# ndpp/ndpp

Hardware: AMD Instinct MI355X
Metric: E_in points*Legendre-orders/sec (free-gas scatter moments) (higher is better)
Workload: dtype f64

## Files before the change

ndpp_amd/csrc/fg_device.h:

```cpp
#pragma once

#include <hip/hip_runtime.h>

#include "fg_pipeline.h"

namespace ndpp {
namespace {

constexpr int kWave = 64;
constexpr int kMuWavesPerSimd = 2;
constexpr int kMuBlocksPerCU = 4 * kMuWavesPerSimd;

struct DevAtomics {
  __device__ static int add(int* p, int v) { return atomicAdd(p, v); }
};

typedef __attribute__((address_space(3))) double lds_f64;
typedef __attribute__((address_space(3))) unsigned lds_u32;

constexpr int mu_stack_fields(int R) { return 2 + 2 * R; }
constexpr int mu_lds_levels(int R) {
  const int budget = (160 * 1024) / kMuBlocksPerCU - 64;
  const int fit = budget / (kWave * (8 * mu_stack_fields(R) + 4));
  return (R == 1 && fit > kStackLdsLevels) ? kStackLdsLevels : fit;
}

template <int R>
struct DevMuStack {
  static constexpr int NF = mu_stack_fields(R);
  lds_f64* lds;
  lds_u32* ldsm;
  char* gbase;
  unsigned goff, gstride;
  int lane, d0;
  static constexpr unsigned kRecBytes = 8u * (NF + 1);
  __device__ __forceinline__ bool in_lds(int d) const { return d >= d0; }
  __device__ __forceinline__ void push(int d, double b, double w, const double* Xb,
                                       const double* Xe, unsigned m) {
    if (in_lds(d)) {
      const int o = __mul24(d - d0, NF * kWave) + lane;
      lds[o] = b; lds[o + kWave] = w;
#pragma unroll
      for (int r = 0; r < R; ++r) {
        lds[o + (2 + r) * kWave] = Xb[r];
        lds[o + (2 + R + r) * kWave] = Xe[r];
      }
      ldsm[(d - d0) * kWave + lane] = m;
    } else {
      double* p = (double*)(gbase + (size_t)(goff + __umul24((unsigned)d, gstride)));
      p[0] = b; p[1] = w;
#pragma unroll
      for (int r = 0; r < R; ++r) { p[2 + r] = Xb[r]; p[2 + R + r] = Xe[r]; }
      *(unsigned*)(p + NF) = m;
    }
  }
  __device__ __forceinline__ void pop(int d, double& b, double& w, double* Xb,
                                      double* Xe, unsigned& m) const {
    if (in_lds(d)) {
      const int o = __mul24(d - d0, NF * kWave) + lane;
      b = lds[o]; w = lds[o + kWave];
#pragma unroll
      for (int r = 0; r < R; ++r) {
        Xb[r] = lds[o + (2 + r) * kWave];
        Xe[r] = lds[o + (2 + R + r) * kWave];
      }
      m = ldsm[(d - d0) * kWave + lane];
    } else {
      const double* p = (const double*)(gbase + (size_t)(goff + __umul24((unsigned)d, gstride)));
      b = p[0]; w = p[1];
#pragma unroll
      for (int r = 0; r < R; ++r) { Xb[r] = p[2 + r]; Xe[r] = p[2 + R + r]; }
      m = *(const unsigned*)(p + NF);
    }
  }
};

__global__ void fg_prep_kernel(FgBatch B, int level) {
  if (*B.overflow) return;
  const int base = B.lvl_off(level);
  const int nt = B.n_tasks(level);
  for (int t = blockIdx.x * blockDim.x + threadIdx.x; t < nt;
       t += gridDim.x * blockDim.x)
    fg_prep_task(B, level, base, t);
}

template <int R, int LMAX, bool kPath>
__device__ __forceinline__ void mu_wave_loop(const FgBatch& B, int level, int base, int nt,
                                             int* counter, DevMuStack<R>& st) {
  MuLane<R, LMAX> s;
  s.mask = 0;
  const PnConsts pk = make_pn_consts<(R * LMAX <= 12 && LMAX <= 8)>();
  bool active = false, more = true;
  bool counts = true;
  unsigned long long n_k = 0, n_v = 0, n_i = 0, n_o = 0;
  unsigned long long w_it = 0, l_it = 0;
  const int kTaskBlock = nt >= (int)(gridDim.x * 16 * kWave) ? 4 * kWave : kWave;
  int blk_next = 0, blk_end = 0;
  constexpr int kFetchMin = kPath ? 8 : 1;
  auto lanes = [](bool x) -> unsigned long long { return __builtin_amdgcn_ballot_w64(x); };
  for (;;) {
    unsigned long long need = more ? lanes(!active) : 0ull;
    if (kFetchMin > 1 && need && __popcll(need) < kFetchMin && lanes(active)) need = 0;
    if (need) {
      if (blk_next >= blk_end) {
        const int first = __ffsll((long long)need) - 1;
        int b = 0;
        if (threadIdx.x == (unsigned)first) b = atomicAdd(counter, kTaskBlock);
        b = __builtin_amdgcn_readlane(b, first);
        blk_next = b;
        blk_end = (b + kTaskBlock < nt) ? b + kTaskBlock : nt;
        if (b >= nt) more = false;
      }
      if (!active && more) {
        const int rank = __popcll(need & ((1ull << threadIdx.x) - 1ull));
        const int t = blk_next + rank;
        if (t < blk_end) {
          if (kPath) mu_init_split<R, LMAX>(B, level, base, t, s);
          else mu_init<R, LMAX>(B, level, base, t, s);
          active = (s.mask != 0);
          if (kPath) counts = (s.path_bits == 0);
          if (active) mu_tot_zero(s);
        }
      }
      const int taken = __popcll(need);
      blk_next = (blk_next + taken < blk_end) ? blk_next + taken : blk_end;
    }
    const unsigned long long act = lanes(active);
    if (!act && !more) break;
    w_it += 1;
    l_it += (unsigned long long)__popcll(act);
    if (active) {
      if (!mu_step<R, LMAX, DevMuStack<R>, kPath>(B, s, st, pk)) {
        mu_finish(B, s, kPath);
        n_k += 2ull * s.visits + 3;
        n_v += s.visits;
        n_o += s.ovisits;
        n_i += counts ? 1 : 0;
        active = false;
      }
    }
  }
  for (int o = 32; o > 0; o >>= 1) {
    n_k += __shfl_down(n_k, o);
    n_v += __shfl_down(n_v, o);
    n_i += __shfl_down(n_i, o);
    n_o += __shfl_down(n_o, o);
  }
  if (threadIdx.x == 0) {
    atomicAdd(&B.stats[kStatKEvals], n_k);
    atomicAdd(&B.stats[kStatMuVisits], n_v);
    atomicAdd(&B.stats[kStatMuIntegrals], n_i);
    atomicAdd(&B.stats[kStatOrderVisits], n_o);
    atomicAdd(&B.stats[kStatWaveIters], w_it);
    atomicAdd(&B.stats[kStatLaneIters], l_it);
  }
}

template <int R, int LMAX>
__global__ __launch_bounds__(kWave, kMuWavesPerSimd) void fg_mu_kernel(FgBatch B, int level, double* gstack, int* counter) {
  constexpr int NF = mu_stack_fields(R), kLevels = mu_lds_levels(R);
  __shared__ double lds[kLevels * NF * kWave];
  __shared__ unsigned ldsm[kLevels * kWave];
  DevMuStack<R> st;
  st.lds = (lds_f64*)lds;
  st.ldsm = (lds_u32*)ldsm;
  st.gbase = (char*)gstack;
  st.goff = (blockIdx.x * kWave + threadIdx.x) * DevMuStack<R>::kRecBytes;
  st.gstride = gridDim.x * kWave * DevMuStack<R>::kRecBytes;
  st.lane = threadIdx.x;
  st.d0 = B.mu_its > kLevels ? B.mu_its - kLevels : 0;

  if (*B.overflow) return;
  const int base = B.lvl_off(level);
  if (B.split_level(level))
    mu_wave_loop<R, LMAX, true>(B, level, base, B.n_mu_tasks(level) * kSplit, counter, st);
  else
    mu_wave_loop<R, LMAX, false>(B, level, base, B.n_mu_tasks(level), counter, st);
}

__global__ void fg_seg_zero_kernel(FgBatch B, int level) {
  if (*B.overflow || !B.split_level(level)) return;
  const size_t n = (size_t)B.n_mu_tasks(level) * kSplit * B.nch();
  for (size_t k = blockIdx.x * (size_t)blockDim.x + threadIdx.x; k < n; k += (size_t)gridDim.x * blockDim.x)
    B.seg[k] = 0.0;
}

__global__ void fg_mu_combine_kernel(FgBatch B, int level) {
  if (*B.overflow || !B.split_level(level)) return;
  const int base = B.lvl_off(level);
  const int nch = B.nch();
  const long tot = (long)B.n_mu_tasks(level) * nch;
  for (long k = blockIdx.x * (long)blockDim.x + threadIdx.x; k < tot; k += (long)gridDim.x * blockDim.x) {
    const int t = (int)(k / nch), ch = (int)(k - (long)t * nch);
    int n, slot;
    fg_task_decode(B, level, base, t, n, slot);
    const unsigned mask = (unsigned)B.node_info[4 * n + 0];
    const int r = ch / B.L, l = ch - r * B.L;
    if (!(mask & chan_bit(r, l))) continue;
    const unsigned gl_rows = B.t_gl ? B.t_gl[B.rec_index(level, base, n, slot)] : 0u;
    if (gl_rows >> r & 1u) continue;
    const double* sg = B.seg + (size_t)t * kSplit * nch + ch;
    double sum = 0.0;
    for (int j = 0; j < kSplit; ++j) sum = sum + sg[(size_t)j * nch];
    B.F(slot, ch, n) = sum;
  }
}

__global__ void fg_setup_kernel(FgBatch B) {
  const int n = B.n_jobs * B.G;
  for (int i = blockIdx.x * blockDim.x + threadIdx.x; i < n;
       i += gridDim.x * blockDim.x)
    fg_setup_group(B, i / B.G, i % B.G);
}

__global__ void fg_node_kernel(FgBatch B, int level) {
  if (*B.overflow) return;
  const int base = B.lvl_off(level);
  const int nn = B.lvl_cnt[level];
  for (int i = blockIdx.x * blockDim.x + threadIdx.x; i < nn;
       i += gridDim.x * blockDim.x)
    fg_node_process<DevAtomics>(B, level, base, i);
  if (blockIdx.x == 0 && threadIdx.x == 0)
    atomicAdd(&B.stats[kStatEoutNodes], (unsigned long long)nn);
}

__global__ void fg_reduce_kernel(FgBatch B, int level) {
  if (*B.overflow) return;
  const int base = B.lvl_off(level);
  const int nn = B.lvl_cnt[level];
  for (int i = blockIdx.x * blockDim.x + threadIdx.x; i < nn;
       i += gridDim.x * blockDim.x)
    fg_reduce_node(B, base, i);
}

__global__ void fg_assemble_kernel(FgBatch B) {
  if (*B.overflow) return;
  const int n_calls = B.n_jobs * B.R;
  for (int c = blockIdx.x * blockDim.x + threadIdx.x; c < n_calls;
       c += gridDim.x * blockDim.x)
    fg_assemble_call(B, c);
}

inline int fg_blocks(long n, int threads = 256) {
  long b = (n + threads - 1) / threads;
  return (int)(b < 1 ? 1 : (b > 4096 ? 4096 : b));
}
inline void launch_fg_setup(const FgBatch& B, hipStream_t s) {
  hipLaunchKernelGGL(fg_setup_kernel, dim3(fg_blocks((long)B.n_jobs * B.G)), dim3(256), 0, s, B);
}
inline void launch_fg_prep(const FgBatch& B, int level, hipStream_t s) {
  hipLaunchKernelGGL(fg_prep_kernel, dim3(2048), dim3(256), 0, s, B, level);
}
inline void launch_fg_seg_zero(const FgBatch& B, int level, hipStream_t s) {
  hipLaunchKernelGGL(fg_seg_zero_kernel, dim3(4096), dim3(256), 0, s, B, level);
}
inline void launch_fg_combine(const FgBatch& B, int level, hipStream_t s) {
  hipLaunchKernelGGL(fg_mu_combine_kernel, dim3(2048), dim3(256), 0, s, B, level);
}
inline void launch_fg_node(const FgBatch& B, int level, hipStream_t s) {
  hipLaunchKernelGGL(fg_node_kernel, dim3(2048), dim3(256), 0, s, B, level);
}
inline void launch_fg_reduce(const FgBatch& B, int level, hipStream_t s) {
  hipLaunchKernelGGL(fg_reduce_kernel, dim3(2048), dim3(256), 0, s, B, level);
}
inline void launch_fg_assemble(const FgBatch& B, hipStream_t s) {
  hipLaunchKernelGGL(fg_assemble_kernel, dim3(fg_blocks((long)B.n_jobs * B.R)), dim3(256), 0, s, B);
}

#if NDPP_FAST
template <int R, int LMAX>
__global__ __launch_bounds__(256) void fg_gauss_kernel(FgBatch B, int level) {
  __shared__ int queue[256 / kWave][2 * kWave];
  if (*B.overflow) return;
  const int base = B.lvl_off(level);
  const int nt = B.n_tasks(level);
  const int lane = threadIdx.x & (kWave - 1);
  int* q = queue[threadIdx.x / kWave];
  int pending = 0;
  unsigned long long nk = 0, ni = 0;
  auto work = [&](int t) {
    const int k = mu_gauss_task<R, LMAX>(B, level, base, t);
    nk += (unsigned long long)k;
    ni += (k > 0 && B.t_gl[t] == (1u << R) - 1u) ? 1ull : 0ull;
  };
  const int stride = gridDim.x * blockDim.x;
  for (int pass = 0; pass < 2; ++pass) {
    for (int t0 = blockIdx.x * blockDim.x + (threadIdx.x - lane); t0 < nt; t0 += stride) {
      const int t = t0 + lane;
      const unsigned flag = t < nt ? B.t_gl[t] : 0u;
      const bool mine = flag != 0 && ((flag & kGaussNear) != 0) == (pass == 1);
      const unsigned long long m = __builtin_amdgcn_ballot_w64(mine);
      if (mine) q[pending + __popcll(m & ((1ull << lane) - 1ull))] = t;
      pending += __popcll(m);
      __builtin_amdgcn_wave_barrier();
      if (pending >= kWave) {
        pending -= kWave;
        const int t1 = q[pending + lane];
        __builtin_amdgcn_wave_barrier();
        work(t1);
      }
    }
    if (lane < pending) work(q[lane]);
    pending = 0;
    __builtin_amdgcn_wave_barrier();
  }
  for (int o = 32; o > 0; o >>= 1) {
    nk += __shfl_down(nk, o);
    ni += __shfl_down(ni, o);
  }
  if (lane == 0 && (nk | ni)) {
    atomicAdd(&B.stats[kStatKEvals], nk);
    atomicAdd(&B.stats[kStatGaussIntegrals], ni);
  }
}
template <int R, int LMAX>
void launch_gauss(const FgBatch& B, int level, hipStream_t s) {
  hipLaunchKernelGGL((fg_gauss_kernel<R, LMAX>), dim3(4096), dim3(256), 0, s, B, level);
}
#endif
void launch_gauss_any(const FgBatch& B, int level, hipStream_t s) {
#if NDPP_FAST
  if (!B.t_gl) return;
  if (B.R == 2) {
    if (B.L <= 4) launch_gauss<2, 4>(B, level, s);
    else if (B.L <= 6) launch_gauss<2, 6>(B, level, s);
    else launch_gauss<2, 8>(B, level, s);
    return;
  }
  if (B.L <= 4) launch_gauss<1, 4>(B, level, s);
  else if (B.L <= 6) launch_gauss<1, 6>(B, level, s);
  else if (B.L <= 8) launch_gauss<1, 8>(B, level, s);
  else launch_gauss<1, 11>(B, level, s);
#else
  (void)B; (void)level; (void)s;
#endif
}

template <int R, int LMAX>
void launch_mu(const FgBatch& B, int level, int num_cu, double* gs, int* counter, hipStream_t s) {
  const int blocks = num_cu * kMuBlocksPerCU;
  hipLaunchKernelGGL((fg_mu_kernel<R, LMAX>), dim3(blocks), dim3(kWave), 0, s, B, level, gs, counter);
}

constexpr int kJointMaxL = 8;

void launch_mu_any(const FgBatch& B, int level, int num_cu, double* gs, int* counter, hipStream_t s) {
  if (B.R == 2) {
    if (B.L <= 4) launch_mu<2, 4>(B, level, num_cu, gs, counter, s);
    else if (B.L <= 6) launch_mu<2, 6>(B, level, num_cu, gs, counter, s);
    else launch_mu<2, 8>(B, level, num_cu, gs, counter, s);
    return;
  }
  if (B.L <= 4) launch_mu<1, 4>(B, level, num_cu, gs, counter, s);
  else if (B.L <= 6) launch_mu<1, 6>(B, level, num_cu, gs, counter, s);
  else if (B.L <= 8) launch_mu<1, 8>(B, level, num_cu, gs, counter, s);
  else launch_mu<1, 11>(B, level, num_cu, gs, counter, s);
}

}
}
```

ndpp_amd/csrc/fg_pipeline.h:

```cpp
#pragma once

#include "ndpp_math.h"

namespace ndpp {
#if NDPP_FAST
inline namespace fast_arith {
#else
inline namespace strict_arith {
#endif

#if NDPP_FAST
constexpr int kMuBlock = 2;
#else
constexpr int kMuBlock = 1;
#endif
constexpr int kSegPerGroup = 5;
constexpr int kMaxLevels = 32;
constexpr int kStackLdsLevels = 8;
constexpr int kMaxRows = 2;
constexpr int kSplitLog2 = 4;
constexpr int kSplit = 1 << kSplitLog2;
constexpr int kRowBits = 16;

enum { kStatKEvals = 0, kStatMuVisits, kStatMuIntegrals, kStatEoutNodes,
       kStatWaveIters, kStatLaneIters, kStatOrderVisits, kStatGaussIntegrals, kNumStats };

NDPP_HD unsigned chan_bit(int r, int l) { return 1u << (r * kRowBits + l); }

struct FgBatch {
  int n_jobs, R, G, L, M;
  double A, kT;
  const double* job_A = nullptr;
  const double* job_kT = nullptr;
  const double* job_ein;
  const int* job_row;
  const double* f_tab;
  const double* e_bins;
  double sab_threshold, brent_thresh, mu_tol, eout_tol;
  int mu_its, eout_its;
  MuGrid grid;
  int ncap;
  double* node_a;
  double* node_b;
  double* node_F;
  double* node_S;
  int* node_info;
  int tcap;
  double* t_mulo;
  double* t_muhi;
  double* t_X;
  unsigned char* t_gl = nullptr;
  double gl_ratio = 2.0;
  int gl_near = 1;
  double gl_amin = 2.0E-6;
  int gl_cert_depth = 7;
  int gl_cert_depth_near = 8;
  int gl_panels = 16;
  int gl_graded = 8;
  int* lvl_cnt;
  int* next_task;
  int* overflow;
  unsigned long long* stats;
  double* seg = nullptr;
  int split_below = 0;
  const int* order = nullptr;
  const int* mask_rank = nullptr;
  const int* mu_nodes = nullptr;
  double* raw;

  NDPP_HD double A_of(int job) const { return job_A ? job_A[job] : A; }
  NDPP_HD double kT_of(int job) const { return job_kT ? job_kT[job] : kT; }
  NDPP_HD int nch() const { return R * L; }
  NDPP_HD int n_trees() const { return n_jobs * G * kSegPerGroup; }
  NDPP_HD int lvl_off(int level) const {
    int o = 0;
    for (int k = 0; k < level; ++k) o += lvl_cnt[k];
    return o;
  }
  NDPP_HD bool split_level(int level) const {
    const int nt = n_mu_tasks(level);
    return seg != nullptr && nt > 0 && nt <= split_below;
  }
  NDPP_HD int tasks_per_node(int level) const { return level == 0 ? 5 : 2; }
  NDPP_HD int n_tasks(int level) const { return lvl_cnt[level] * tasks_per_node(level); }
  NDPP_HD int n_mu_tasks(int level) const {
    return (mu_nodes ? *mu_nodes : lvl_cnt[level]) * tasks_per_node(level);
  }
  NDPP_HD int rec_index(int level, int base, int n, int slot) const {
    return level == 0 ? 5 * n + slot : 2 * (n - base) + (slot == 3 ? 1 : 0);
  }
  NDPP_HD double& F(int slot, int ch, int n) const {
    return node_F[((size_t)(slot * R * L + ch)) * ncap + n];
  }
  NDPP_HD double& S(int ch, int n) const { return node_S[(size_t)ch * ncap + n]; }
  NDPP_HD double& tX(int k, int r, int t) const { return t_X[((size_t)(k * R + r)) * tcap + t]; }
  NDPP_HD unsigned full_mask() const {
    unsigned m = 0;
    for (int r = 0; r < R; ++r) m |= ((1u << L) - 1u) << (r * kRowBits);
    return m;
  }
  NDPP_HD int node_job(int n) const { return node_info[4 * n + 2] & 0x3ffffff; }
  NDPP_HD int node_depth(int n) const { return node_info[4 * n + 2] >> 26; }
};

NDPP_HD void fg_setup_group(const FgBatch& B, int job, int g) {
  const double Ein = B.job_ein[job];
  const double A = B.A_of(job), kT = B.kT_of(job);
  double alphaEin = (A - 1.0) / (A + 1.0);
  alphaEin = alphaEin * alphaEin * Ein;
  double Eout_lo, Eout_hi;
  fg_eout_bounds(A, kT, Ein, Eout_lo, Eout_hi);
  const double eg = B.e_bins[g], eg1 = B.e_bins[g + 1];

  double sa[kSegPerGroup], sb[kSegPerGroup];
  bool on[kSegPerGroup] = {false, false, false, false, false};
  if ((eg < Eout_hi) && (eg1 > Eout_lo)) {
    double Elo = (Eout_lo > eg) ? Eout_lo : eg;
    double Ehi = (Eout_hi < eg1) ? Eout_hi : eg1;
    double Ebottom = (eg == 0.0) ? 0.01 * Elo : eg;
    sa[0] = Ebottom; sb[0] = Elo; on[0] = true;
    sa[1] = Ehi;     sb[1] = eg1; on[1] = true;
    if ((Elo < alphaEin) && (alphaEin < Ehi)) {
      sa[2] = Elo; sb[2] = alphaEin; on[2] = true;
      Elo = alphaEin;
    }
    if ((Elo < Ein) && (Ein < Ehi)) {
      sa[3] = Elo; sb[3] = Ein; on[3] = true;
      Elo = Ein;
    }
    sa[4] = Elo; sb[4] = Ehi; on[4] = true;
  } else {
    sa[4] = eg; sb[4] = eg1; on[4] = true;
  }
  const unsigned full = B.full_mask();
  const int nch = B.nch();
  for (int s = 0; s < kSegPerGroup; ++s) {
    int n = (job * B.G + g) * kSegPerGroup + s;
    bool live = on[s] && (sa[s] != sb[s]);
    B.node_a[n] = live ? sa[s] : 0.0;
    B.node_b[n] = live ? sb[s] : 0.0;
    B.node_info[4 * n + 0] = live ? (int)full : 0;
    B.node_info[4 * n + 1] = -1;
    B.node_info[4 * n + 2] = job;
    B.node_info[4 * n + 3] = 0;
    for (int ch = 0; ch < nch; ++ch) B.S(ch, n) = 0.0;
  }
}

NDPP_HD void fg_task_decode(const FgBatch& B, int level, int base, int t, int& n,
                            int& slot) {
  (void)B;
  int idx;
  if (level == 0) {
    idx = t / 5;
    slot = t - 5 * idx;
  } else {
    idx = t >> 1;
    slot = 1 + 2 * (t & 1);
  }
  n = B.order ? B.order[idx] : (level == 0 ? idx : base + idx);
}

NDPP_HD unsigned fg_sort_key(const FgBatch& B, unsigned mask) {
  unsigned m = 0;
  for (int r = 0; r < B.R; ++r) m |= (mask >> (r * kRowBits)) & ((1u << B.L) - 1u);
  return m;
}

constexpr int kSortClasses = 4;
NDPP_HD int fg_node_bucket(const FgBatch& B, int level, int base, int n, int nb) {
  const unsigned mask = (unsigned)B.node_info[4 * n + 0];
  const int last = kSortClasses * nb - 1;
  if (mask == 0) return last;
  double wmax = -1.0;
  const int nslots = B.tasks_per_node(level);
  for (int k = 0; k < nslots; ++k) {
    const int slot = level == 0 ? k : 1 + 2 * k;
    const int rec = B.rec_index(level, base, n, slot);
    unsigned m = mask;
    if (B.t_gl) {
      const unsigned rows = B.t_gl[rec];
      for (int r = 0; r < B.R; ++r)
        if (rows >> r & 1u) m &= ~(((1u << kRowBits) - 1u) << (r * kRowBits));
    }
    if (m == 0) continue;
    const double km = fmax(fmax(fabs(B.tX(0, 0, rec)), fabs(B.tX(1, 0, rec))), fabs(B.tX(2, 0, rec)));
    const double w = (B.t_muhi[rec] - B.t_mulo[rec]) * km;
    wmax = fmax(wmax, w >= 0.0 ? w : 0.0);
  }
  if (wmax < 0.0) return last;
  const int cls = wmax >= 1073741824.0 ? 0 : wmax >= 1048576.0 ? 1 : wmax >= 256.0 ? 2 : 3;
  int b = cls * nb + B.mask_rank[fg_sort_key(B, mask)];
  return b < last ? b : last - 1;
}

NDPP_HD double fg_slot_point(double a, double b, int slot) {
  double c = 0.5 * (a + b);
  switch (slot) {
    case 0: return a;
    case 1: return 0.5 * (a + c);
    case 2: return c;
    case 3: return 0.5 * (c + b);
    default: return b;
  }
}

template <int R>
NDPP_HD void fg_Krows(const FgPair& q, const MuGrid& g, const double* const* f, double mu,
                      double* K) {
#if NDPP_FAST
  const double E = fg_E(q, mu);
#pragma unroll
  for (int r = 0; r < R; ++r) K[r] = (q.C1 * fg_fval(g, f[r], mu)) * E;
#else
  fg_K_rows<R>(q, g, f, mu, K);
#endif
}
NDPP_HD double simpson(double w, double f0, double f1, double f2) {
  return w * (fma(4.0, f1, f0) + f2);
}

constexpr unsigned kGaussNear = 0x80u;
NDPP_HD unsigned fg_gauss_zone(const FgBatch& B, const FgPair& q, double Ein, double Eout) {
  const double amin = (q.EpE - 2.0 * q.s2) / q.AkT;
  if (!(amin >= B.gl_amin)) return 0u;
  const unsigned rows = (1u << B.R) - 1u;
  if (Eout >= B.gl_ratio * Ein || Ein >= B.gl_ratio * Eout) return rows;
  return B.gl_near ? (rows | kGaussNear) : 0u;
}

NDPP_HD void fg_prep_task(const FgBatch& B, int level, int base, int t) {
  int n, slot;
  if (level == 0) { n = t / 5; slot = t - 5 * n; }
  else { n = base + (t >> 1); slot = 1 + 2 * (t & 1); }
  if (B.node_info[4 * n + 0] == 0) {
    if (B.t_gl) B.t_gl[t] = 0;
    return;
  }
  const int job = B.node_job(n);
  const double Ein = B.job_ein[job];
  const double Eout = fg_slot_point(B.node_a[n], B.node_b[n], slot);
  const double A = B.A_of(job);
  const FgPair q = make_pair(A, B.kT_of(job), Ein, Eout);
  double mlo, mhi;
  fg_find_mu(q, A, Ein, Eout, B.sab_threshold, B.brent_thresh, mlo, mhi);
  const double mc = (mlo + mhi) * 0.5;
  B.t_mulo[t] = mlo;
  B.t_muhi[t] = mhi;
  if (B.t_gl) B.t_gl[t] = (unsigned char)fg_gauss_zone(B, q, Ein, Eout);
  for (int r = 0; r < B.R; ++r) {
    const double* fr[1] = {B.f_tab + (size_t)B.job_row[(size_t)job * B.R + r] * B.M};
    fg_Krows<1>(q, B.grid, fr, mlo, &B.tX(0, r, t));
    fg_Krows<1>(q, B.grid, fr, mhi, &B.tX(1, r, t));
    fg_Krows<1>(q, B.grid, fr, mc, &B.tX(2, r, t));
  }
}

#if NDPP_FAST
constexpr int kGaussN = 16;
NDPP_HD double gauss_node(int j) {
  constexpr double x[kGaussN] = {
      -0.98940093499164994, -0.9445750230732326, -0.86563120238783176, -0.755404408355003,
      -0.61787624440264377, -0.45801677765722737, -0.28160355077925892, -0.095012509837637454,
      0.095012509837637454, 0.28160355077925892, 0.45801677765722737, 0.61787624440264377,
      0.755404408355003, 0.86563120238783176, 0.9445750230732326, 0.98940093499164994};
  return x[j];
}
NDPP_HD double gauss_weight(int j) {
  constexpr double w[kGaussN] = {
      0.027152459411754037, 0.062253523938647706, 0.095158511682492591, 0.12462897125553403,
      0.14959598881657676, 0.16915651939500262, 0.18260341504492361, 0.18945061045506859,
      0.18945061045506859, 0.18260341504492361, 0.16915651939500262, 0.14959598881657676,
      0.12462897125553403, 0.095158511682492591, 0.062253523938647706, 0.027152459411754037};
  return w[j];
}

template <int R, int LMAX, bool kAdd = false>
NDPP_HD void gauss_composite(const FgBatch& B, const FgPair& q, const FView<R>& fv, double a, double b,
                             int panels, const PnConsts& pk, double* acc) {
  if (!kAdd) {
#pragma unroll
    for (int ch = 0; ch < R * LMAX; ++ch) acc[ch] = 0.0;
  }
  const double h = (b - a) / (double)(2 * panels);
  for (int p = 0; p < panels; ++p) {
    const double c = a + h * (double)(2 * p + 1);
    for (int j = 0; j < kGaussN; j += 2) {
      const double mu0 = fma(h, gauss_node(j), c), mu1 = fma(h, gauss_node(j + 1), c);
      FvLoad v0[R], v1[R];
      fg_fval_load_rows<R>(B.grid, fv, mu0, v0);
      fg_fval_load_rows<R>(B.grid, fv, mu1, v1);
      double E0, E1;
      fg_E2(q, mu0, mu1, E0, E1);
      E0 *= h * gauss_weight(j);
      E1 *= h * gauss_weight(j + 1);
      double P0[LMAX], P1[LMAX];
      pn_all<LMAX>(mu0, P0, pk);
      pn_all<LMAX>(mu1, P1, pk);
#pragma unroll
      for (int r = 0; r < R; ++r) {
        const double K0 = (q.C1 * fg_fval_use(v0[r])) * E0;
        const double K1 = (q.C1 * fg_fval_use(v1[r])) * E1;
#pragma unroll
        for (int l = 0; l < LMAX; ++l) acc[r * LMAX + l] = fma(K1, P1[l], fma(K0, P0[l], acc[r * LMAX + l]));
      }
    }
  }
}

template <int R, int LMAX>
NDPP_HD void gauss_graded(const FgBatch& B, const FgPair& q, const FView<R>& fv, double a, double b,
                          int m, int split, const PnConsts& pk, double* acc) {
#pragma unroll
  for (int ch = 0; ch < R * LMAX; ++ch) acc[ch] = 0.0;
  const double W = b - a;
  double lo = a;
  for (int k = 1; k <= m + 1; ++k) {
    const double hi = k <= m ? b - ldexp(W, -k) : b;
    gauss_composite<R, LMAX, true>(B, q, fv, lo, hi, split, pk, acc);
    lo = hi;
  }
}

constexpr double kGaussAgree = 1.0E-13;
constexpr int kCertDepth = 5;
constexpr double kCertBig = 64.0;

template <int R, int LMAX>
NDPP_HD unsigned mu_gauss_certify(const FgBatch& B, const FgPair& q, const FView<R>& fv, int t, unsigned mask,
                                  unsigned rows, int cert_depth, const PnConsts& pk) {
  const double a = B.t_mulo[t], b = B.t_muhi[t];
  auto Kat = [&](double mu0, double mu1, double* K0, double* K1) {
    FvLoad v0[R], v1[R];
    fg_fval_load_rows<R>(B.grid, fv, mu0, v0);
    fg_fval_load_rows<R>(B.grid, fv, mu1, v1);
    double E0, E1;
    fg_E2(q, mu0, mu1, E0, E1);
#pragma unroll
    for (int r = 0; r < R; ++r) {
      K0[r] = (q.C1 * fg_fval_use(v0[r])) * E0;
      K1[r] = (q.C1 * fg_fval_use(v1[r])) * E1;
    }
  };
  for (int dep = 0; dep < cert_depth; ++dep) {
    const int nn = 1 << dep;
    const double hd = (b - a) / (double)nn;
    const double w = hd * (1.0 / 12.0);
    const double wp = dep == 0 ? hd / 6.0 : (2.0 * hd) * (1.0 / 12.0);
    const double eps15 = 15.0 * ldexp(B.mu_tol, -dep);
    const bool strict = dep < kCertDepth;
    const double big15 = kCertBig * eps15;
    unsigned prev_leaf = 0, prev_big = 0;
    double Ka[R], Pa[LMAX];
#pragma unroll
    for (int r = 0; r < R; ++r) Ka[r] = B.tX(0, r, t);
    pn_all<LMAX>(a, Pa, pk);
    for (int j = 0; j < nn; ++j) {
      const double xa = a + hd * (double)j;
      const double xb = (j == nn - 1) ? b : a + hd * (double)(j + 1);
      const double xc = 0.5 * (xa + xb), xd = 0.5 * (xa + xc), xe = 0.5 * (xc + xb);
      double Kd[R], Ke[R], Kc[R], Kb[R];
      Kat(xd, xe, Kd, Ke);
      Kat(xc, xb, Kc, Kb);
      if (dep == 0) {
#pragma unroll
        for (int r = 0; r < R; ++r) { Kc[r] = B.tX(2, r, t); Kb[r] = B.tX(1, r, t); }
      } else if (j == nn - 1) {
#pragma unroll
        for (int r = 0; r < R; ++r) Kb[r] = B.tX(1, r, t);
      }
      double Pd[LMAX], Pc[LMAX], Pe[LMAX], Pb[LMAX];
      pn_all<LMAX>(xd, Pd, pk); pn_all<LMAX>(xc, Pc, pk); pn_all<LMAX>(xe, Pe, pk); pn_all<LMAX>(xb, Pb, pk);
      unsigned leaf = 0, big = 0;
#pragma unroll
      for (int r = 0; r < R; ++r) {
        const double Xc2 = 2.0 * Kc[r], Xc4 = 4.0 * Kc[r], Kd4 = 4.0 * Kd[r], Ke4 = 4.0 * Ke[r];
#pragma unroll
        for (int l = 0; l < LMAX; ++l) {
          const double T = fma(Kb[r], Pb[l], Ka[r] * Pa[l]);
          const double s1 = fma(Xc4, Pc[l], T);
          const double s2 = fma(Ke4, Pe[l], fma(Kd4, Pd[l], fma(Xc2, Pc[l], T)));
          const double dS = fabs(fma(w, s2, -(wp * s1)));
          if (mask & chan_bit(r, l)) {
            if (!(dS > eps15)) leaf |= chan_bit(r, l);
            if (dS > big15) big |= chan_bit(r, l);
          }
        }
      }
      const unsigned bad = strict ? leaf : ((leaf & prev_big) | (prev_leaf & big));
#pragma unroll
      for (int r = 0; r < R; ++r)
        if (bad & (((1u << kRowBits) - 1u) << (r * kRowBits))) rows &= ~(1u << r);
      if (rows == 0) return 0;
      prev_leaf = leaf;
      prev_big = big;
#pragma unroll
      for (int r = 0; r < R; ++r) Ka[r] = Kb[r];
#pragma unroll
      for (int l = 0; l < LMAX; ++l) Pa[l] = Pb[l];
    }
  }
  return rows;
}

template <int R, int LMAX>
NDPP_HD int mu_gauss_task(const FgBatch& B, int level, int base, int t) {
  unsigned rows = B.t_gl[t];
  if (!rows) return 0;
  const bool near = (rows & kGaussNear) != 0;
  const int cert_depth = near ? B.gl_cert_depth_near : B.gl_cert_depth;
  rows &= ~kGaussNear;
  int n_node, slot;
  if (level == 0) { n_node = t / 5; slot = t - 5 * n_node; }
  else { n_node = base + (t >> 1); slot = 1 + 2 * (t & 1); }
  const unsigned mask = (unsigned)B.node_info[4 * n_node + 0];
#pragma unroll
  for (int r = 0; r < R; ++r)
    if (!(mask & (((1u << kRowBits) - 1u) << (r * kRowBits)))) rows &= ~(1u << r);
  if (rows == 0) { B.t_gl[t] = 0; return 0; }
  const int job = B.node_job(n_node);
  const double Ein = B.job_ein[job];
  const double Eout = fg_slot_point(B.node_a[n_node], B.node_b[n_node], slot);
  const FgPair q = make_pair(B.A_of(job), B.kT_of(job), Ein, Eout);
  FRows f;
  f.off = 8u * (unsigned)B.M * (unsigned)B.job_row[(size_t)job * R];
  const FView<R> fv = f_view<R>(B.f_tab, f, B.M);
  const double a = B.t_mulo[t], b = B.t_muhi[t];
  const PnConsts pk = make_pn_consts();
  rows = mu_gauss_certify<R, LMAX>(B, q, fv, t, mask, rows, cert_depth, pk);
  if (rows == 0) {
    B.t_gl[t] = 0;
    return 4 * ((1 << cert_depth) - 1);
  }
  double Ic[R * LMAX], If[R * LMAX];
  int evals = 4 * ((1 << cert_depth) - 1);
  unsigned done = 0;
  auto take_agreeing_rows = [&]() {
#pragma unroll
    for (int r = 0; r < R; ++r) {
      if (!((rows & ~done) >> r & 1u)) continue;
      bool ok = true;
#pragma unroll
      for (int l = 0; l < LMAX; ++l)
        ok = ok && (fabs(If[r * LMAX + l] - Ic[r * LMAX + l]) <= kGaussAgree * fabs(If[r * LMAX]));
      if (!ok) continue;
      done |= 1u << r;
#pragma unroll
      for (int l = 0; l < LMAX; ++l)
        if (l < B.L && (mask & chan_bit(r, l))) B.F(slot, r * B.L + l, n_node) = If[r * LMAX + l];
    }
  };
  if (near && B.gl_graded > 0) {
    gauss_graded<R, LMAX>(B, q, fv, a, b, B.gl_graded, 1, pk, Ic);
    gauss_graded<R, LMAX>(B, q, fv, a, b, B.gl_graded, 2, pk, If);
    evals += 3 * (B.gl_graded + 1) * kGaussN;
    take_agreeing_rows();
    if (done == rows) {
      B.t_gl[t] = (unsigned char)rows;
      return evals;
    }
  }
  gauss_composite<R, LMAX>(B, q, fv, a, b, 4, pk, Ic);
  evals += 4 * kGaussN;
  for (int n = 8;; n *= 2) {
    gauss_composite<R, LMAX>(B, q, fv, a, b, n, pk, If);
    evals += n * kGaussN;
    take_agreeing_rows();
    if (done == rows || 2 * n > B.gl_panels) break;
#pragma unroll
    for (int k = 0; k < R * LMAX; ++k) Ic[k] = If[k];
  }
  rows = done;
  B.t_gl[t] = (unsigned char)rows;
  return evals;
}
#endif

template <int R, int LMAX>
struct MuLane {
  static constexpr int NCH = R * LMAX;
  static constexpr unsigned kChanMask = []() {
    unsigned m = 0;
    for (int r = 0; r < R; ++r) m |= (LMAX >= 32 ? ~0u : ((1u << LMAX) - 1u)) << (r * kRowBits);
    return m;
  }();
  FgPair q;
  FRows f;
  double a, b;
  double wp;
  double Xc[R], Xb[R];
  double fa[NCH];
  double acc[NCH];
  double tot[NCH];
  int path_left, own_from;
  unsigned path_bits;
  bool own_pending;
  unsigned slot_path;
  int task;
  unsigned chans;
  unsigned mask;
  unsigned pending;
  int depth;
  int node, slot;
  unsigned visits, ovisits;
};

template <int R, int LMAX>
NDPP_HD void mu_tot_zero(MuLane<R, LMAX>& s) {
#pragma unroll
  for (int ch = 0; ch < R * LMAX; ++ch) s.tot[ch] = 0.0;
}

template <int R>
struct HostMuStack {
  double b[kMaxLevels], w[kMaxLevels], Xb[kMaxLevels][R], Xe[kMaxLevels][R];
  unsigned m[kMaxLevels];
  NDPP_HD void push(int d, double b_, double w_, const double* Xb_, const double* Xe_, unsigned m_) {
    b[d] = b_; w[d] = w_; m[d] = m_;
    for (int r = 0; r < R; ++r) { Xb[d][r] = Xb_[r]; Xe[d][r] = Xe_[r]; }
  }
  NDPP_HD void pop(int d, double& b_, double& w_, double* Xb_, double* Xe_, unsigned& m_) const {
    b_ = b[d]; w_ = w[d]; m_ = m[d];
    for (int r = 0; r < R; ++r) { Xb_[r] = Xb[d][r]; Xe_[r] = Xe[d][r]; }
  }
};

NDPP_HD int highest_bit(unsigned x) {
#if defined(__HIP_DEVICE_COMPILE__)
  return 31 - __clz((int)x);
#else
  return 31 - __builtin_clz(x);
#endif
}

NDPP_HD int popcount32(unsigned x) {
#if defined(__HIP_DEVICE_COMPILE__)
  return __popc(x);
#else
  return __builtin_popcount(x);
#endif
}

template <int R, int LMAX>
NDPP_HD void mu_init(const FgBatch& B, int level, int base, int t, MuLane<R, LMAX>& s) {
  int n, slot;
  fg_task_decode(B, level, base, t, n, slot);
  s.node = n;
  s.slot = slot;
  s.mask = (unsigned)B.node_info[4 * n + 0] & MuLane<R, LMAX>::kChanMask;
  s.pending = 0;
  s.depth = 0;
  s.visits = 0;
  s.ovisits = 0;
#pragma unroll
  for (int ch = 0; ch < R * LMAX; ++ch) s.acc[ch] = 0.0;
  s.path_left = 0; s.own_from = 0; s.path_bits = 0; s.own_pending = false; s.slot_path = 0;
  s.task = t;
  s.chans = s.mask;
  if (s.mask == 0) return;
  const int rec = B.rec_index(level, base, n, slot);
  if (B.t_gl) {
    const unsigned rows = B.t_gl[rec];
#pragma unroll
    for (int r = 0; r < R; ++r)
      if (rows >> r & 1u) s.mask &= ~(((1u << kRowBits) - 1u) << (r * kRowBits));
    s.chans = s.mask;
    if (s.mask == 0) return;
  }
  const int job = B.node_job(n);
  const double Ein = B.job_ein[job];
  const double Eout = fg_slot_point(B.node_a[n], B.node_b[n], slot);
  s.q = make_pair(B.A_of(job), B.kT_of(job), Ein, Eout);
  s.f.off = 8u * (unsigned)B.M * (unsigned)B.job_row[(size_t)job * R];
  s.a = B.t_mulo[rec];
  s.b = B.t_muhi[rec];
  double Xa[R];
#pragma unroll
  for (int r = 0; r < R; ++r) {
    Xa[r] = B.tX(0, r, rec);
    s.Xb[r] = B.tX(1, r, rec);
    s.Xc[r] = B.tX(2, r, rec);
  }
  const double h = s.b - s.a;
  s.wp = h / 6.0;
  double Pa[LMAX];
  pn_all<LMAX>(s.a, Pa, make_pn_consts());
#pragma unroll
  for (int r = 0; r < R; ++r)
#pragma unroll
    for (int l = 0; l < LMAX; ++l) s.fa[r * LMAX + l] = Xa[r] * Pa[l];
}

template <int R, int LMAX, class Stack, bool kPath = true>
NDPP_HD bool mu_step(const FgBatch& B, MuLane<R, LMAX>& s, Stack& st, const PnConsts& pk) {
  if (kPath && s.own_pending && s.depth == s.own_from) {
    s.own_pending = false;
#pragma unroll
    for (int ch = 0; ch < R * LMAX; ++ch) s.acc[ch] = 0.0;
    mu_tot_zero(s);
  }
  const double c = 0.5 * (s.a + s.b);
  const double h = s.b - s.a;
  const double d = 0.5 * (s.a + c);
  const double e = 0.5 * (c + s.b);
  const int dj_top = s.pending ? highest_bit(s.pending) : (B.mu_its > 0 ? B.mu_its - 1 : 0);
  int dj = dj_top;
  double bj, wj, Xbj[R], Xej[R];
  unsigned mj;
  st.pop(dj, bj, wj, Xbj, Xej, mj);
  double Kd[R], Ke[R];
#if NDPP_FAST
  {
    FvLoad fvd[R], fve[R];
    const FView<R> fv = f_view<R>(B.f_tab, s.f, B.M);
    fg_fval_load_rows<R>(B.grid, fv, d, fvd);
    fg_fval_load_rows<R>(B.grid, fv, e, fve);
#if defined(__HIP_DEVICE_COMPILE__)
    __builtin_amdgcn_sched_barrier(0);
#endif
    double Ed, Ee;
    fg_E2(s.q, d, e, Ed, Ee);
#pragma unroll
    for (int r = 0; r < R; ++r) {
      Kd[r] = (s.q.C1 * fg_fval_use(fvd[r])) * Ed;
      Ke[r] = (s.q.C1 * fg_fval_use(fve[r])) * Ee;
    }
  }
  const double w = h * (1.0 / 12.0);
  double Xc2[R], Xc4[R], Kd4[R], Ke4[R];
#pragma unroll
  for (int r = 0; r < R; ++r) {
    Xc2[r] = 2.0 * s.Xc[r]; Xc4[r] = 4.0 * s.Xc[r];
    Kd4[r] = 4.0 * Kd[r]; Ke4[r] = 4.0 * Ke[r];
  }
#else
  fg_K_rows_pair<R>(s.q, B.grid, f_view<R>(B.f_tab, s.f, B.M), d, e, Kd, Ke);
  const double w = div_by<12>(h);
#endif
  const bool bottom = (B.mu_its - s.depth) <= 0;
  const double eps15 = bottom ? 1.7976931348623157e308 * 2.0 : 15.0 * ldexp(B.mu_tol, -s.depth);
  double Pd[LMAX], Pc[LMAX], Pe[LMAX], Pb[LMAX];
  pn_all<LMAX>(d, Pd, pk);
  pn_all<LMAX>(c, Pc, pk);
  pn_all<LMAX>(e, Pe, pk);
  pn_all<LMAX>(s.b, Pb, pk);
  unsigned refine = 0;
#pragma unroll
  for (int l0 = 0; l0 < LMAX; l0 += kMuBlock) {
    unsigned any = 0;
#pragma unroll
    for (int l = l0; l < l0 + kMuBlock && l < LMAX; ++l)
#pragma unroll
      for (int r = 0; r < R; ++r) any |= s.mask & chan_bit(r, l);
    if (!any) continue;
#pragma unroll
    for (int l = l0; l < l0 + kMuBlock && l < LMAX; ++l) {
#pragma unroll
      for (int r = 0; r < R; ++r) {
        const int ch = r * LMAX + l;
        constexpr bool kAlone = (R == 1 && kMuBlock == 1);
        const bool active = kAlone || (s.mask & chan_bit(r, l)) != 0;
        const double fa = s.fa[ch];
#if NDPP_FAST
        const double T = fma(s.Xb[r], Pb[l], fa);
        const double s1 = fma(Xc4[r], Pc[l], T);
        const double s2 = fma(Ke4[r], Pe[l], fma(Kd4[r], Pd[l], fma(Xc2[r], Pc[l], T)));
        const double S = s.wp * s1;
        const double dS = fma(w, s2, -S);
        const double v = fma(dS, 16.0 / 15.0, S);
#else
        const double fd = Kd[r] * Pd[l];
        const double fc = s.Xc[r] * Pc[l];
        const double fe = Ke[r] * Pe[l];
        const double fb = s.Xb[r] * Pb[l];
        const double S = opaque(simpson(s.wp, fa, fc, fb));
        const double S2 = simpson(w, fa, fd, fc) + simpson(w, fc, fe, fb);
        const double dS = S2 - S;
        const double v = fma(dS, 1.0 / 15.0, S2);
#endif
        const bool leaf = !(fabs(dS) > eps15);
        if (kAlone) {
          if (leaf) s.acc[ch] = s.acc[ch] + v;
          else refine |= chan_bit(r, l);
        } else {
#if defined(__HIP_DEVICE_COMPILE__)
          {
            const unsigned long long am = __builtin_amdgcn_ballot_w64((s.mask & chan_bit(r, l)) != 0);
            const unsigned long long lm = __builtin_amdgcn_ballot_w64(!(fabs(dS) > eps15));
            const unsigned long long tm = am & lm, rm = am & ~lm;
            unsigned long long sv;
            unsigned rb;
            asm("s_and_saveexec_b64 %[sv], %[tm]\n\t"
                "v_add_f64 %[a], %[a], %[v]\n\t"
                "s_mov_b64 exec, %[sv]"
                : [sv] "=&s"(sv), [a] "+v"(s.acc[ch])
                : [tm] "s"(tm), [v] "v"(v)
                : "scc");
            asm("v_cndmask_b32_e64 %[rb], 0, %[bit], %[rm]" : [rb] "=v"(rb) : [bit] "v"(chan_bit(r, l)), [rm] "s"(rm));
            refine |= rb;
          }
#else
          s.acc[ch] = (active && leaf) ? s.acc[ch] + v : s.acc[ch];
          refine |= (active && !leaf) ? chan_bit(r, l) : 0u;
#endif
        }
      }
    }
  }
  s.visits += 1;
  s.ovisits += (unsigned)popcount32(s.mask);
  bool resume = false;
  if (refine) {
    bool go_right = false;
    if (kPath && s.path_left > 0) {
      s.path_left -= 1;
      go_right = ((s.path_bits >> s.path_left) & 1u) != 0;
      if (!go_right) {
        s.b = c;
#pragma unroll
        for (int r = 0; r < R; ++r) { s.Xb[r] = s.Xc[r]; s.Xc[r] = Kd[r]; }
        s.wp = w;
        s.mask = refine;
        s.depth += 1;
        return true;
      }
    }
    if (go_right) {
      dj = s.depth; bj = s.b; wj = w; mj = refine;
#pragma unroll
      for (int r = 0; r < R; ++r) { Xbj[r] = s.Xb[r]; Xej[r] = Ke[r]; s.Xb[r] = s.Xc[r]; }
      s.b = c;
      resume = true;
    } else {
      st.push(s.depth, s.b, w, s.Xb, Ke, refine);
      s.pending |= 1u << s.depth;
      s.b = c;
#pragma unroll
      for (int r = 0; r < R; ++r) { s.Xb[r] = s.Xc[r]; s.Xc[r] = Kd[r]; }
      s.wp = w;
      s.mask = refine;
      s.depth += 1;
      return true;
    }
  }
  if (resume || s.pending) {
    s.pending &= ~(1u << dj);
    if (dj + 1 <= kSplitLog2) {
      if constexpr (kPath) {
        if (!s.own_pending) {
          const unsigned nmask = (unsigned)B.node_info[4 * s.node + 0];
#pragma unroll
          for (int r = 0; r < R; ++r)
#pragma unroll
            for (int l = 0; l < LMAX; ++l)
              if (nmask & chan_bit(r, l))
                B.seg[((size_t)s.task * kSplit + s.slot_path) * B.nch() + r * B.L + l] = s.acc[r * LMAX + l];
        }
#pragma unroll
        for (int ch = 0; ch < R * LMAX; ++ch) s.acc[ch] = 0.0;
        s.slot_path = (s.slot_path & ~((1u << (kSplitLog2 - dj)) - 1u)) | (1u << (kSplitLog2 - dj - 1));
      } else {
#pragma unroll
        for (int ch = 0; ch < R * LMAX; ++ch) {
          s.tot[ch] = s.tot[ch] + s.acc[ch];
          s.acc[ch] = 0.0;
        }
      }
    }
    s.a = s.b;
    {
      double Pa[LMAX];
      if (kPath && resume) {
        pn_all<LMAX>(s.a, Pa, pk);
      } else {
#pragma unroll
        for (int l = 0; l < LMAX; ++l) Pa[l] = Pb[l];
      }
#pragma unroll
      for (int r = 0; r < R; ++r)
#pragma unroll
        for (int l = 0; l < LMAX; ++l) s.fa[r * LMAX + l] = s.Xb[r] * Pa[l];
    }
    s.b = bj;
#pragma unroll
    for (int r = 0; r < R; ++r) { s.Xb[r] = Xbj[r]; s.Xc[r] = Xej[r]; }
    s.wp = wj;
    s.mask = mj;
    s.depth = dj + 1;
    return true;
  }
  return false;
}

template <int R, int LMAX>
NDPP_HD void mu_finish(const FgBatch& B, const MuLane<R, LMAX>& s, bool split = false) {
  const unsigned mask = s.chans;
#pragma unroll
  for (int r = 0; r < R; ++r)
#pragma unroll
    for (int l = 0; l < LMAX; ++l)
      if (mask & chan_bit(r, l)) {
        if (split) {
          if (!s.own_pending)
            B.seg[((size_t)s.task * kSplit + s.slot_path) * B.nch() + r * B.L + l] = s.acc[r * LMAX + l];
          continue;
        }
        B.F(s.slot, r * B.L + l, s.node) = s.tot[r * LMAX + l] + s.acc[r * LMAX + l];
      }
}

template <int R, int LMAX>
NDPP_HD void mu_init_split(const FgBatch& B, int level, int base, int t, MuLane<R, LMAX>& s) {
  const int nt = B.n_mu_tasks(level);
  const int i = t % nt, rank = t / nt;
  mu_init<R, LMAX>(B, level, base, i, s);
  int jp = 0;
  if (s.mask != 0) {
#if NDPP_FAST
    const double pa = s.q.p, qa = s.q.q;
#else
    const double pa = s.q.EpE / s.q.AkT, qa = 2.0 * s.q.s2 / s.q.AkT;
#endif
    const double x = ((pa - fabs(s.q.beta)) / qa - s.a) / (s.b - s.a) * (double)kSplit;
    jp = (x > 0.0) ? (x < (double)(kSplit - 1) ? (int)x : kSplit - 1) : 0;
  }
  int lo = jp - 1, hi = jp, cur = hi;
  for (int k = 0; k <= rank; ++k) {
    if (((k & 1) == 0 && hi < kSplit) || lo < 0) cur = hi++;
    else cur = lo--;
  }
  s.path_left = kSplitLog2;
  s.path_bits = (unsigned)cur;
  s.slot_path = 0;
  int tz = 0;
  while (tz < kSplitLog2 && !(((unsigned)cur >> tz) & 1u)) ++tz;
  s.own_from = kSplitLog2 - tz;
  s.own_pending = (s.own_from != 0);
}

NDPP_HD void fg_mu_combine_task(const FgBatch& B, int level, int base, int t) {
  int n, slot;
  fg_task_decode(B, level, base, t, n, slot);
  const unsigned mask = (unsigned)B.node_info[4 * n + 0];
  if (mask == 0) return;
  const unsigned gl_rows = B.t_gl ? B.t_gl[B.rec_index(level, base, n, slot)] : 0u;
  const int nch = B.nch();
  for (int r = 0; r < B.R; ++r)
    for (int l = 0; l < B.L; ++l)
      if ((mask & chan_bit(r, l)) && !(gl_rows >> r & 1u)) {
        const int ch = r * B.L + l;
        double tot = 0.0;
        for (int j = 0; j < kSplit; ++j) tot = tot + B.seg[((size_t)t * kSplit + j) * nch + ch];
        B.F(slot, ch, n) = tot;
      }
}

struct HostAtomics {
  static int add(int* p, int v) { int o = *p; *p += v; return o; }
};

template <class Atomics>
NDPP_HD void fg_node_process(const FgBatch& B, int level, int base, int i) {
  const int n = base + i;
  const unsigned mask = (unsigned)B.node_info[4 * n + 0];
  if (mask == 0) return;
  const int depth = B.node_depth(n);
  const double a = B.node_a[n], b = B.node_b[n];
  const double c = 0.5 * (a + b);
  const double h = b - a;
  const double w = h / 12.0;
  const double eps15 = 15.0 * ldexp(B.eout_tol, -depth);
  const bool bottom = (B.eout_its - depth) <= 0;
  unsigned refine = 0;
  auto half = [w](double f0, double f1, double f2) { return w * (f0 + 4.0 * f1 + f2); };
  for (int r = 0; r < B.R; ++r)
    for (int l = 0; l < B.L; ++l) {
      if (!(mask & chan_bit(r, l))) continue;
      const int ch = r * B.L + l;
      const double Fa = B.F(0, ch, n), Fd = B.F(1, ch, n), Fc = B.F(2, ch, n),
                   Fe = B.F(3, ch, n), Fb = B.F(4, ch, n);
      double S = B.S(ch, n);
      if (depth == 0) S = (h / 6.0) * (Fa + 4.0 * Fc + Fb);
      const double S2 = half(Fa, Fd, Fc) + half(Fc, Fe, Fb);
      if (bottom || (fabs(S2 - S) <= eps15)) {
        B.S(ch, n) = S2 + (S2 - S) / 15.0;
      } else {
        refine |= chan_bit(r, l);
      }
    }
  B.node_info[4 * n + 3] = (int)refine;
  if (!refine) return;
  const int pos = Atomics::add(&B.lvl_cnt[level + 1], 2);
  const int left = base + B.lvl_cnt[level] + pos;
  if (left + 2 > B.ncap) {
    *B.overflow = 1;
    B.node_info[4 * n + 3] = 0;
    return;
  }
  B.node_info[4 * n + 1] = left;
  const int job = B.node_job(n);
  for (int k = 0; k < 2; ++k) {
    const int m = left + k;
    B.node_a[m] = k ? c : a;
    B.node_b[m] = k ? b : c;
    B.node_info[4 * m + 0] = (int)refine;
    B.node_info[4 * m + 1] = -1;
    B.node_info[4 * m + 2] = job | ((depth + 1) << 26);
    B.node_info[4 * m + 3] = 0;
    for (int r = 0; r < B.R; ++r)
      for (int l = 0; l < B.L; ++l) {
        if (!(refine & chan_bit(r, l))) continue;
        const int ch = r * B.L + l;
        const double f0 = B.F(k ? 2 : 0, ch, n), f1 = B.F(k ? 3 : 1, ch, n), f2 = B.F(k ? 4 : 2, ch, n);
        B.F(0, ch, m) = f0;
        B.F(2, ch, m) = f1;
        B.F(4, ch, m) = f2;
        B.S(ch, m) = half(f0, f1, f2);
      }
  }
}

NDPP_HD void fg_reduce_node(const FgBatch& B, int base, int i) {
  const int n = base + i;
  const unsigned refine = (unsigned)B.node_info[4 * n + 3];
  if (!refine) return;
  const int left = B.node_info[4 * n + 1];
  for (int r = 0; r < B.R; ++r)
    for (int l = 0; l < B.L; ++l)
      if (refine & chan_bit(r, l)) {
        const int ch = r * B.L + l;
        B.S(ch, n) = B.S(ch, left) + B.S(ch, left + 1);
      }
}

NDPP_HD void fg_assemble_call(const FgBatch& B, int call) {
  const int L = B.L, G = B.G;
  const int job = call / B.R, r = call - job * B.R;
  double* out = B.raw + (size_t)call * G * L;
  double p0 = 0.0;
  for (int g = 0; g < G; ++g) {
    const int root = (job * G + g) * kSegPerGroup;
    for (int l = 0; l < L; ++l) {
      const int ch = r * L + l;
      double v = B.S(ch, root + 0) + B.S(ch, root + 1);
      v = v + B.S(ch, root + 2);
      v = v + B.S(ch, root + 3);
      v = v + B.S(ch, root + 4);
      out[g * L + l] = v;
    }
    p0 = p0 + out[g * L + 0];
    for (int l = 0; l < L; ++l)
      if (fabs(out[g * L + l]) < 1.0E-18) out[g * L + l] = 0.0;
  }
  for (int k = 0; k < G * L; ++k) out[k] = out[k] / p0;
}

}
}
```

Measured before the change: 284,700.

## Cut register pressure in Gauss quadrature kernel via LDS stash and per-order Legendre evaluation

Moves the coarse-estimate accumulator array Ic into LDS (strided per thread), raises the launch-bounds occupancy hint for small channel counts, and evaluates Legendre polynomials one order at a time instead of materialising full P arrays. The graded and composite refinement paths are merged into one loop, and the node loop is kept rolled. The aim is to lower VGPR usage so more waves fit per SIMD. The cost is extra LDS traffic, possible recomputation in per-order Legendre evaluation, and possible spills if the occupancy hint forces too few registers.

```diff
diff --git a/ndpp_amd/csrc/fg_device.h b/ndpp_amd/csrc/fg_device.h
--- a/ndpp_amd/csrc/fg_device.h
+++ b/ndpp_amd/csrc/fg_device.h
@@ -268,9 +268,16 @@
 }
 
 #if NDPP_FAST
+struct GaussIcLds {
+  lds_f64* p;
+  __device__ __forceinline__ lds_f64& operator[](int k) const { return p[k * 256]; }
+};
+constexpr int gauss_waves_per_simd(int R, int LMAX) { return (R * LMAX <= 12 && LMAX <= 8) ? 3 : 2; }
 template <int R, int LMAX>
-__global__ __launch_bounds__(256) void fg_gauss_kernel(FgBatch B, int level) {
+__global__ __launch_bounds__(256, gauss_waves_per_simd(R, LMAX)) void fg_gauss_kernel(FgBatch B, int level) {
   __shared__ int queue[256 / kWave][2 * kWave];
+  __shared__ double ic[R * LMAX * 256];
+  const GaussIcLds ic_lane{(lds_f64*)ic + threadIdx.x};
   if (*B.overflow) return;
   const int base = B.lvl_off(level);
   const int nt = B.n_tasks(level);
@@ -279,7 +286,7 @@
   int pending = 0;
   unsigned long long nk = 0, ni = 0;
   auto work = [&](int t) {
-    const int k = mu_gauss_task<R, LMAX>(B, level, base, t);
+    const int k = mu_gauss_task<R, LMAX>(B, level, base, t, ic_lane);
     nk += (unsigned long long)k;
     ni += (k > 0 && B.t_gl[t] == (1u << R) - 1u) ? 1ull : 0ull;
   };
diff --git a/ndpp_amd/csrc/fg_pipeline.h b/ndpp_amd/csrc/fg_pipeline.h
--- a/ndpp_amd/csrc/fg_pipeline.h
+++ b/ndpp_amd/csrc/fg_pipeline.h
@@ -1,4 +1,6 @@
 #pragma once
+
+#include <type_traits>
 
 #include "ndpp_math.h"
 
@@ -275,6 +277,20 @@
   return w[j];
 }
 
+template <int l>
+NDPP_HD double pn_value(double x, const PnConsts& k) {
+  double v;
+  pn_range<l, 1>(x, &v, k);
+  return v;
+}
+template <int N, int I = 0, class F>
+NDPP_HD void static_for(F&& f) {
+  if constexpr (I < N) {
+    f(std::integral_constant<int, I>{});
+    static_for<N, I + 1>(f);
+  }
+}
+
 template <int R, int LMAX, bool kAdd = false>
 NDPP_HD void gauss_composite(const FgBatch& B, const FgPair& q, const FView<R>& fv, double a, double b,
                              int panels, const PnConsts& pk, double* acc) {
@@ -285,6 +301,7 @@
   const double h = (b - a) / (double)(2 * panels);
   for (int p = 0; p < panels; ++p) {
     const double c = a + h * (double)(2 * p + 1);
+#pragma unroll 1
     for (int j = 0; j < kGaussN; j += 2) {
       const double mu0 = fma(h, gauss_node(j), c), mu1 = fma(h, gauss_node(j + 1), c);
       FvLoad v0[R], v1[R];
@@ -294,16 +311,18 @@
       fg_E2(q, mu0, mu1, E0, E1);
       E0 *= h * gauss_weight(j);
       E1 *= h * gauss_weight(j + 1);
-      double P0[LMAX], P1[LMAX];
-      pn_all<LMAX>(mu0, P0, pk);
-      pn_all<LMAX>(mu1, P1, pk);
+      double K0[R], K1[R];
 #pragma unroll
       for (int r = 0; r < R; ++r) {
-        const double K0 = (q.C1 * fg_fval_use(v0[r])) * E0;
-        const double K1 = (q.C1 * fg_fval_use(v1[r])) * E1;
-#pragma unroll
-        for (int l = 0; l < LMAX; ++l) acc[r * LMAX + l] = fma(K1, P1[l], fma(K0, P0[l], acc[r * LMAX + l]));
-      }
+        K0[r] = (q.C1 * fg_fval_use(v0[r])) * E0;
+        K1[r] = (q.C1 * fg_fval_use(v1[r])) * E1;
+      }
+      static_for<LMAX>([&](auto lc) {
+        constexpr int l = decltype(lc)::value;
+        const double P0 = pn_value<l>(mu0, pk), P1 = pn_value<l>(mu1, pk);
+#pragma unroll
+        for (int r = 0; r < R; ++r) acc[r * LMAX + l] = fma(K1[r], P1, fma(K0[r], P0, acc[r * LMAX + l]));
+      });
     }
   }
 }
@@ -369,24 +388,29 @@
 #pragma unroll
         for (int r = 0; r < R; ++r) Kb[r] = B.tX(1, r, t);
       }
-      double Pd[LMAX], Pc[LMAX], Pe[LMAX], Pb[LMAX];
-      pn_all<LMAX>(xd, Pd, pk); pn_all<LMAX>(xc, Pc, pk); pn_all<LMAX>(xe, Pe, pk); pn_all<LMAX>(xb, Pb, pk);
+      double Xc2[R], Xc4[R], Kd4[R], Ke4[R];
+#pragma unroll
+      for (int r = 0; r < R; ++r) {
+        Xc2[r] = 2.0 * Kc[r]; Xc4[r] = 4.0 * Kc[r]; Kd4[r] = 4.0 * Kd[r]; Ke4[r] = 4.0 * Ke[r];
+      }
       unsigned leaf = 0, big = 0;
-#pragma unroll
-      for (int r = 0; r < R; ++r) {
-        const double Xc2 = 2.0 * Kc[r], Xc4 = 4.0 * Kc[r], Kd4 = 4.0 * Kd[r], Ke4 = 4.0 * Ke[r];
-#pragma unroll
-        for (int l = 0; l < LMAX; ++l) {
-          const double T = fma(Kb[r], Pb[l], Ka[r] * Pa[l]);
-          const double s1 = fma(Xc4, Pc[l], T);
-          const double s2 = fma(Ke4, Pe[l], fma(Kd4, Pd[l], fma(Xc2, Pc[l], T)));
+      static_for<LMAX>([&](auto lc) {
+        constexpr int l = decltype(lc)::value;
+        const double Pd = pn_value<l>(xd, pk), Pc = pn_value<l>(xc, pk);
+        const double Pe = pn_value<l>(xe, pk), Pb = pn_value<l>(xb, pk);
+#pragma unroll
+        for (int r = 0; r < R; ++r) {
+          const double T = fma(Kb[r], Pb, Ka[r] * Pa[l]);
+          const double s1 = fma(Xc4[r], Pc, T);
+          const double s2 = fma(Ke4[r], Pe, fma(Kd4[r], Pd, fma(Xc2[r], Pc, T)));
           const double dS = fabs(fma(w, s2, -(wp * s1)));
           if (mask & chan_bit(r, l)) {
             if (!(dS > eps15)) leaf |= chan_bit(r, l);
             if (dS > big15) big |= chan_bit(r, l);
           }
         }
-      }
+        Pa[l] = Pb;
+      });
       const unsigned bad = strict ? leaf : ((leaf & prev_big) | (prev_leaf & big));
 #pragma unroll
       for (int r = 0; r < R; ++r)
@@ -396,15 +420,13 @@
       prev_big = big;
 #pragma unroll
       for (int r = 0; r < R; ++r) Ka[r] = Kb[r];
-#pragma unroll
-      for (int l = 0; l < LMAX; ++l) Pa[l] = Pb[l];
     }
   }
   return rows;
 }
 
-template <int R, int LMAX>
-NDPP_HD int mu_gauss_task(const FgBatch& B, int level, int base, int t) {
+template <int R, int LMAX, class IcStash>
+NDPP_HD int mu_gauss_task(const FgBatch& B, int level, int base, int t, IcStash Ic) {
   unsigned rows = B.t_gl[t];
   if (!rows) return 0;
   const bool near = (rows & kGaussNear) != 0;
@@ -432,7 +454,7 @@
     B.t_gl[t] = 0;
     return 4 * ((1 << cert_depth) - 1);
   }
-  double Ic[R * LMAX], If[R * LMAX];
+  double If[R * LMAX];
   int evals = 4 * ((1 << cert_depth) - 1);
   unsigned done = 0;
   auto take_agreeing_rows = [&]() {
@@ -450,29 +472,36 @@
         if (l < B.L && (mask & chan_bit(r, l))) B.F(slot, r * B.L + l, n_node) = If[r * LMAX + l];
     }
   };
-  if (near && B.gl_graded > 0) {
-    gauss_graded<R, LMAX>(B, q, fv, a, b, B.gl_graded, 1, pk, Ic);
-    gauss_graded<R, LMAX>(B, q, fv, a, b, B.gl_graded, 2, pk, If);
-    evals += 3 * (B.gl_graded + 1) * kGaussN;
-    take_agreeing_rows();
-    if (done == rows) {
-      B.t_gl[t] = (unsigned char)rows;
-      return evals;
-    }
-  }
-  gauss_composite<R, LMAX>(B, q, fv, a, b, 4, pk, Ic);
-  evals += 4 * kGaussN;
-  for (int n = 8;; n *= 2) {
-    gauss_composite<R, LMAX>(B, q, fv, a, b, n, pk, If);
-    evals += n * kGaussN;
-    take_agreeing_rows();
-    if (done == rows || 2 * n > B.gl_panels) break;
+  int m = (near && B.gl_graded > 0) ? B.gl_graded : 0;
+  int n = m > 0 ? 1 : 4;
+  bool compare = false;
+  for (;;) {
+    gauss_graded<R, LMAX>(B, q, fv, a, b, m, n, pk, If);
+    evals += (m + 1) * n * kGaussN;
+    if (compare) {
+      take_agreeing_rows();
+      if (done == rows) break;
+      if (m > 0) {
+        m = 0;
+        n = 4;
+        compare = false;
+        continue;
+      }
+      if (2 * n > B.gl_panels) break;
+    }
 #pragma unroll
     for (int k = 0; k < R * LMAX; ++k) Ic[k] = If[k];
+    compare = true;
+    n *= 2;
   }
   rows = done;
   B.t_gl[t] = (unsigned char)rows;
   return evals;
+}
+template <int R, int LMAX>
+NDPP_HD int mu_gauss_task(const FgBatch& B, int level, int base, int t) {
+  double Ic[R * LMAX];
+  return mu_gauss_task<R, LMAX>(B, level, base, t, Ic);
 }
 #endif
 
```

New measurement: 287,200 (median of 6 runs). Within noise of the previous version (+0.9%).
